# CFSAN-Biostatistics/snp-pipeline

Hardware: AMD Instinct MI355X
Metric: consensus_bases_called_per_sec (higher is better)
Workload: dtype u8; 1 GPU; BASELINE configs[3] shard (125 samples/GPU x 5000000 bp x 30x synthetic pileups, 49878 SNP sites, 1500 SNP records per sample; the reference bundles no pileups); step = site-record gather + site union, one batched scan launch + one call launch, 4-bit pack, row all-gather, all-pairs distance tiles, row-band exchange; samples_total=125, samples_this_rank=125, genome_bp=5000000, snp_sites=49878, pileup_bytes_this_rank=54061520755, parallelism=samples sharded over 1 rank(s)

## Files before the change

### include/snpgpu.h

```cpp
#ifndef SNPGPU_H
#define SNPGPU_H

#include <stddef.h>
#include <stdint.h>

#ifdef __cplusplus
extern "C" {
#endif

#define SNPGPU_ABI_VERSION 7

#define SNPGPU_OK            0
#define SNPGPU_E_HIP        -1
#define SNPGPU_E_ARG        -2
#define SNPGPU_E_NOMEM      -3
#define SNPGPU_E_PILEUP     -4
#define SNPGPU_E_UNSUPPORTED -5
#define SNPGPU_E_IO         -6
#define SNPGPU_E_TIMEOUT    -7

#define SNPGPU_F_RAWDPTH  0x01
#define SNPGPU_F_VARFREQ  0x02
#define SNPGPU_F_DEPTH    0x04
#define SNPGPU_F_STRDPTH  0x08
// ... 474 lines not shown
int  snpgpu_tiles_gather_dev(snpgpu_ctx *ctx, const int32_t *d_matrix, uint32_t n_padded, const uint32_t *d_tile_rows,
                             const uint32_t *d_tile_cols, uint32_t n_tiles, int32_t *d_out);
int  snpgpu_tiles_scatter_dev(snpgpu_ctx *ctx, const int32_t *d_tiles, const uint32_t *d_tile_rows, const uint32_t *d_tile_cols,
                              uint32_t n_tiles, int32_t *d_matrix, uint32_t n_padded);
int  snpgpu_group_check_dev(snpgpu_ctx *ctx, const uint8_t *d_filters, const snpgpu_site_counts *d_counts, const uint64_t *d_line_off,
                            const uint8_t *d_wanted, const uint32_t *d_excl_off, const uint32_t *d_excl_slots,
                            uint32_t n_samples, uint32_t n_sites, int64_t *d_out);

int  snpgpu_dense_windows(snpgpu_ctx *ctx, const int64_t *positions, const uint32_t *seg_off, uint32_t n_segs,
                          const int32_t *max_snps, const int32_t *window, uint32_t n_rules,
                          int64_t *out_start, int64_t *out_end, uint32_t *out_seg, uint32_t *out_n);
int  snpgpu_dense_windows_dev(snpgpu_ctx *ctx, const int64_t *d_positions, const uint32_t *d_seg_off, uint32_t n_segs,
                              uint32_t n_pos, const int32_t *max_snps , const int32_t *window ,
                              uint32_t n_rules, int64_t *d_out_start, int64_t *d_out_end, uint32_t *d_out_seg,
                              uint32_t *d_out_n );
int  snpgpu_merge_regions(snpgpu_ctx *ctx, const uint32_t *group, const int64_t *start, const int64_t *end,
                          uint32_t n, uint32_t *out_group, int64_t *out_start, int64_t *out_end, uint32_t *out_n);
int  snpgpu_merge_regions_dev(snpgpu_ctx *ctx, const uint32_t *d_group, const int64_t *d_start, const int64_t *d_end,
                              uint32_t n, uint32_t *d_out_group, int64_t *d_out_start, int64_t *d_out_end,
                              uint32_t *d_out_n );
int  snpgpu_in_regions(snpgpu_ctx *ctx, const uint32_t *pos_group, const int64_t *positions, uint32_t n_pos,
                       const uint32_t *reg_off, const int64_t *reg_start, const int64_t *reg_end,
                       uint32_t n_groups, uint8_t *out_flag);
int  snpgpu_in_regions_dev(snpgpu_ctx *ctx, const uint32_t *d_pos_group, const int64_t *d_positions, uint32_t n_pos,
                           const uint32_t *d_reg_off, const int64_t *d_reg_start, const int64_t *d_reg_end,
                           uint32_t n_groups, uint8_t *d_out_flag);

int  snpgpu_merge_sites(snpgpu_ctx *ctx, const uint64_t *keys, const uint32_t *sample_of_key, size_t n,
                        uint64_t *out_unique, uint32_t *out_off, uint32_t *out_carrier,
                        uint32_t *out_n_unique, uint32_t *out_n_carrier);
int  snpgpu_merge_sites_dev(snpgpu_ctx *ctx, const uint64_t *d_keys, const uint32_t *d_sample_of_key, uint32_t n,
                            uint64_t *d_out_unique, uint32_t *d_out_off, uint32_t *d_out_carrier,
                            uint32_t *d_out_n );

typedef struct snpgpu_synth_params {
    uint64_t seed;
    uint32_t sample;
    uint32_t genome_len;
    float    mean_depth;
    float    carrier_p_same_clade;
    float    carrier_p_other_clade;
    uint32_t n_clades;
    char     contig[32];
} snpgpu_synth_params;
int  snpgpu_synth_reference_dev(snpgpu_ctx *ctx, uint64_t seed, uint32_t genome_len, uint8_t *d_ref );
int  snpgpu_synth_pileup_dev(snpgpu_ctx *ctx, const snpgpu_synth_params *p, const uint8_t *d_ref,
                             const uint8_t *d_site_alt, uint8_t *d_out, size_t capacity, size_t *out_nbytes);

#define SNPGPU_BGZF_E_NOT_GZIP   -101
#define SNPGPU_BGZF_E_NOT_BGZF   -102
#define SNPGPU_BGZF_E_TRUNCATED  -103
#define SNPGPU_BGZF_E_ISIZE      -104
#define SNPGPU_BGZF_E_MAGIC      -105
#define SNPGPU_BGZF_ST_OK           0
#define SNPGPU_BGZF_ST_BTYPE        1
#define SNPGPU_BGZF_ST_STORED_LEN   2
#define SNPGPU_BGZF_ST_CODE_SET     3
#define SNPGPU_BGZF_ST_SYMBOL       4
#define SNPGPU_BGZF_ST_DISTANCE     5
#define SNPGPU_BGZF_ST_INPUT_END    6
#define SNPGPU_BGZF_ST_OUTPUT_OVER  7
#define SNPGPU_BGZF_ST_OUTPUT_SHORT 8
#define SNPGPU_BGZF_ST_CRC          9
typedef struct snpgpu_bgzf_block {
    uint64_t coff;
    uint64_t poff;
// ... 36 lines not shown
```

### snp_pipeline_amd/_lib.py

```python
import ctypes as C
import os

_HERE = os.path.dirname(os.path.abspath(__file__))
LIB_PATH = os.path.join(_HERE, "lib", "libsnpgpu.so")

MAX_SYMS = 8
SCAN_STATUS_WORDS = 4
CALL_PASSES = 4

F_RAWDPTH, F_VARFREQ, F_DEPTH, F_STRDPTH, F_STRBIAS, F_REGION = 1, 2, 4, 8, 16, 32
SITE_IN_SNPLIST, SITE_EXCLUDED = 1, 2
ST_NO_LINE, ST_OK, ST_SHORT_LINE, ST_BAD_DEPTH, ST_NO_QUALS, ST_MULTI_REF = 0, 1, 2, 3, 4, 5
VCF_LINE_WINDOW, VCF_MORE_UNUSUAL, VCF_LONG_LINE = 4096, 1, 2
E_HIP, E_ARG, E_NOMEM, E_PILEUP, E_UNSUPPORTED, E_IO, E_TIMEOUT = -1, -2, -3, -4, -5, -6, -7


class CallerParams(C.Structure):
    _fields_ = [("min_base_quality", C.c_int32), ("min_cons_depth", C.c_int32),
                ("min_cons_strand_depth", C.c_int32), ("reserved", C.c_int32),
                ("min_cons_freq", C.c_double), ("min_cons_strand_bias", C.c_double)]


class SiteCounts(C.Structure):
    _fields_ = [("raw_depth", C.c_uint32), ("good_depth", C.c_uint32), ("fwd_good_depth", C.c_uint32),
# ... 194 lines not shown
                                          C.c_int]),
    "snpgpu_pair_sites_kept": (C.c_int, [_P, _P, _P, C.c_uint64, C.c_uint64, _P, _P, _P, C.POINTER(C.c_uint64)]),
    "snpgpu_packed_drop": (C.c_int, [_P]),
    "snpgpu_write_pair_sites_tsv": (C.c_int, [C.c_char_p, _P, _P, C.c_uint32, _P, _P, C.c_uint64, _P, _P, _P, _P, _P, _P, _P]),
    "snpgpu_distance_rect_packed_dev": (C.c_int, [_P, _P, C.c_uint32, _P, C.c_uint32, C.c_uint32, C.c_int, _P, C.c_uint64]),
    "snpgpu_nearest_dev": (C.c_int, [_P, _P, C.c_uint32, C.c_uint32, C.c_uint64, C.c_uint32, C.c_int32, C.c_uint64, _P, _P, _P, C.POINTER(C.c_uint64)]),
    "snpgpu_nearest": (C.c_int, [_P, _P, C.c_uint32, _P, C.c_uint32, C.c_uint32, C.c_uint32, C.c_int32, C.c_uint32, C.c_int, C.c_uint64, _P, _P, _P,
                                 C.POINTER(C.c_uint64), _P]),
    "snpgpu_write_nearest_tsv": (C.c_int, [C.c_char_p, _P, _P, C.c_uint32, _P, _P, C.c_uint32, _P, _P, _P]),
    "snpgpu_valid_plane_row_bytes": (C.c_size_t, [C.c_uint32]),
    "snpgpu_valid_plane_dev": (C.c_int, [_P, _P, C.c_uint32, C.c_uint32, _P]),
    "snpgpu_compared_rect_dev": (C.c_int, [_P, _P, C.c_uint32, _P, C.c_uint32, C.c_uint32, _P, C.c_uint64]),
    "snpgpu_compared_pairs_dev": (C.c_int, [_P, _P, C.c_uint32, _P, C.c_uint32, C.c_uint32, _P, _P, C.c_uint64, _P]),
    "snpgpu_compared": (C.c_int, [_P, _P, C.c_uint32, C.c_uint32, _P]),
    "snpgpu_compared_pairs": (C.c_int, [_P, _P, C.c_uint32, _P, C.c_uint32, C.c_uint32, _P, _P, C.c_uint64, _P]),
    "snpgpu_write_pair_rows_tsv": (C.c_int, [C.c_char_p, _P, _P, C.c_uint32, _P, _P, C.c_uint32, _P, _P, _P, _P, C.c_uint64]),
    "snpgpu_site_counts_dev": (C.c_int, [_P, _P, C.c_uint32, C.c_uint32, _P]),
    "snpgpu_site_counts_host": (C.c_int, [_P, _P, C.c_uint32, C.c_uint32, _P]),
    "snpgpu_cluster_snps_dev": (C.c_int, [_P, _P, C.c_uint32, C.c_uint32, _P, C.c_uint32, C.c_uint64, _P, _P, _P, _P, C.POINTER(C.c_uint64)]),
    "snpgpu_cluster_snps": (C.c_int, [_P, _P, C.c_uint32, C.c_uint32, _P, _P, C.c_uint32, C.c_uint64, _P, _P, _P, _P, C.POINTER(C.c_uint64)]),
    "snpgpu_write_site_counts_tsv": (C.c_int, [C.c_char_p, _P, C.c_uint32, C.c_uint32, _P, _P, _P, _P]),
    "snpgpu_write_cluster_snps_tsv": (C.c_int, [C.c_char_p, _P, _P, C.c_uint32, _P, _P, _P, _P, _P, C.c_uint32, _P, _P, _P, _P]),
    "snpgpu_dense_windows": (C.c_int, [_P, _P, _P, C.c_uint32, _P, _P, C.c_uint32, _P, _P, _P, C.POINTER(C.c_uint32)]),
    "snpgpu_merge_regions": (C.c_int, [_P, _P, _P, _P, C.c_uint32, _P, _P, _P, C.POINTER(C.c_uint32)]),
    "snpgpu_in_regions": (C.c_int, [_P, _P, _P, C.c_uint32, _P, _P, _P, C.c_uint32, _P]),
    "snpgpu_merge_sites": (C.c_int, [_P, _P, _P, C.c_size_t, _P, _P, _P, C.POINTER(C.c_uint32), C.POINTER(C.c_uint32)]),
    "snpgpu_dense_windows_dev": (C.c_int, [_P, _P, _P, C.c_uint32, C.c_uint32, _P, _P, C.c_uint32, _P, _P, _P, _P]),
    "snpgpu_merge_regions_dev": (C.c_int, [_P, _P, _P, _P, C.c_uint32, _P, _P, _P, _P]),
    "snpgpu_in_regions_dev": (C.c_int, [_P, _P, _P, C.c_uint32, _P, _P, _P, C.c_uint32, _P]),
    "snpgpu_merge_vcf_files": (C.c_int, [_P, C.POINTER(C.c_char_p), C.c_uint32, C.c_char_p, C.c_char_p, C.c_uint32, C.c_uint32, _P]),
    "snpgpu_merge_vcf_files_opts": (C.c_int, [_P, C.POINTER(C.c_char_p), C.c_uint32, C.c_char_p, C.c_char_p, C.c_uint32, _P, _P, _P]),
    "snpgpu_merge_plan": (C.c_int, [C.c_uint32, C.c_uint64, C.c_uint64, _P, _P]),
    "snpgpu_merge_sites_dev": (C.c_int, [_P, _P, _P, C.c_uint32, _P, _P, _P, _P]),
    "snpgpu_comm_available": (C.c_int, []),
    "snpgpu_comm_version": (C.c_int, [C.POINTER(C.c_int)]),
    "snpgpu_comm_unique_id": (C.c_int, [_P]),
    "snpgpu_comm_init": (C.c_int, [_P, C.c_int, C.c_int, _P]),
    "snpgpu_comm_destroy": (None, [_P]),
    "snpgpu_comm_abort": (None, [_P]),
    "snpgpu_comm_info": (C.c_int, [_P, C.POINTER(C.c_int), C.POINTER(C.c_int), C.POINTER(C.c_int)]),
    "snpgpu_allgather": (C.c_int, [_P, _P, _P, C.c_size_t]),
    "snpgpu_allgatherv": (C.c_int, [_P, _P, _P, _P, _P]),
    "snpgpu_alltoallv": (C.c_int, [_P, _P, _P, _P, _P]),
    "snpgpu_stream_wait": (C.c_int, [_P, C.c_uint32]),
    "snpgpu_tiles_gather_dev": (C.c_int, [_P, _P, C.c_uint32, _P, _P, C.c_uint32, _P]),
    "snpgpu_tiles_scatter_dev": (C.c_int, [_P, _P, _P, _P, C.c_uint32, _P, C.c_uint32]),
    "snpgpu_group_check_dev": (C.c_int, [_P, _P, _P, _P, _P, _P, _P, C.c_uint32, C.c_uint32, _P]),
    "snpgpu_synth_reference_dev": (C.c_int, [_P, C.c_uint64, C.c_uint32, _P]),
    "snpgpu_synth_pileup_dev": (C.c_int, [_P, C.POINTER(SynthParams), _P, _P, _P, C.c_size_t, C.POINTER(C.c_size_t)]),
    "snpgpu_bgzf_probe": (C.c_int, [C.c_char_p]),
    "snpgpu_bgzf_strerror": (C.c_char_p, [C.c_int]),
    "snpgpu_bgzf_status_name": (C.c_char_p, [C.c_uint32]),
    "snpgpu_bgzf_index": (C.c_int, [_P, C.c_uint64, _P, C.c_uint64, C.POINTER(C.c_uint64), C.POINTER(BgzfInfo)]),
    "snpgpu_bgzf_inflate_dev": (C.c_int, [_P, _P, C.c_uint64, _P, C.c_uint64, _P, C.c_uint64, _P, C.POINTER(BgzfInfo)]),
    "snpgpu_bgzf_inflate_block_host": (C.c_uint32, [_P, C.POINTER(BgzfBlock), _P]),
    "snpgpu_bgzf_read_range": (C.c_int, [C.c_char_p, C.c_uint64, C.c_uint64, _P, C.POINTER(C.c_uint64)]),
    "snpgpu_call_consensus_bgzf_files": (C.c_int, [_P, _P, C.POINTER(C.c_char_p), C.c_uint32, C.POINTER(CallerParams), _P, _P, _P, _P,
                                                   _P, _P, _P, _P, C.POINTER(StreamOpts), C.POINTER(StreamStats), _P]),
}

_lib = None


class SnpGpuError(RuntimeError):
    def __init__(self, code, message):
        RuntimeError.__init__(self, "snpgpu error %d: %s" % (code, message))
# ... 27 lines not shown
```

### snp_pipeline_amd/csrc/regions.hip

```cpp
#include <string.h>

#include <vector>

#include "internal.h"
#include "prims.h"

namespace {

inline size_t up256(size_t x) { return (x + 255) / 256 * 256; }
inline unsigned nblk(uint64_t n) { return (unsigned)((n + 255) / 256); }

#define R_TRY(ctx, expr)                                                                                \
    do {                                                                                                \
        hipError_t e_ = (expr);                                                                         \
        if (e_ != hipSuccess)                                                                           \
            return snpgpu_set_error((ctx), SNPGPU_E_HIP, "%s failed: %s", #expr, hipGetErrorString(e_)); \
    } while (0)

#define REG_ERR_POSITION 1u
#define REG_ERR_INTERVAL 2u

struct U64Less { __device__ bool operator()(const uint64_t &a, const uint64_t &b) const { return a < b; } };

#define MAX_RULES 64
struct Rules { int32_t max_snps[MAX_RULES], window[MAX_RULES]; uint32_t n; };

__device__ __forceinline__ uint32_t seg_of(const uint32_t *seg_off, uint32_t n_segs, uint32_t i) {
    uint32_t lo = 0, hi = n_segs;
    while (hi - lo > 1) { uint32_t mid = (lo + hi) >> 1; if (seg_off[mid] <= i) lo = mid; else hi = mid; }
    return lo;
}

// ... 146 lines not shown
        k_ival_pack<<<nblk(n), 256, 0, st>>>(d_group, d_start, d_end, n, iv, d_out_n);
        const Ival *sorted = prim_sort<Ival, IvalLess>(st, iv, ia, ib, n, sflag, IvalLess());
        k_ival_ends<<<nblk(n), 256, 0, st>>>(sorted, n, gm);
        prim_inclusive_scan<GroupMax, GroupMaxOp>(st, gm, run, n, aggr, GroupMaxOp());
        k_ival_heads<<<nblk(n), 256, 0, st>>>(sorted, run, n, head);
        uint32_t *d_total = nullptr;
        prim_exclusive_scan_u32(st, head, slot, n, scan_ws, &d_total);
        k_ival_emit<<<nblk(n), 256, 0, st>>>(sorted, run, head, slot, n, d_out_group, d_out_start, d_out_end);
        k_copy_word<<<1, 1, 0, st>>>(d_total, d_out_n);
    }
    R_TRY(ctx, hipGetLastError());
    return SNPGPU_OK;
}

__global__ void k_in_regions(const uint32_t *pos_group, const int64_t *pos, uint32_t n, const uint32_t *reg_off,
                             const int64_t *rs, const int64_t *re, uint32_t n_groups, uint8_t *out) {
    uint32_t i = blockIdx.x * blockDim.x + threadIdx.x;
    if (i >= n) return;
    uint32_t g = pos_group[i];
    uint8_t f = 0;
    if (g < n_groups) {
        int64_t p = pos[i];
        uint32_t lo = reg_off[g], hi = reg_off[g + 1];
        while (lo < hi) {
            uint32_t mid = (lo + hi) >> 1;
            if (rs[mid] <= p) lo = mid + 1; else hi = mid;
        }
        if (lo > reg_off[g]) f = re[lo - 1] >= p;
    }
    out[i] = f;
}

struct Pair { uint64_t key; uint32_t samp, pad; };
struct PairLess {
    __device__ bool operator()(const Pair &a, const Pair &b) const { return a.key != b.key ? a.key < b.key : a.samp < b.samp; }
};

__global__ void k_pair_pack(const uint64_t *keys, const uint32_t *samp, uint32_t n, Pair *out) {
    uint32_t i = blockIdx.x * blockDim.x + threadIdx.x;
    if (i < n) { Pair p; p.key = keys[i]; p.samp = samp[i]; p.pad = 0; out[i] = p; }
}

__global__ void k_sites_flags(const Pair *sorted, uint32_t n, uint32_t *new_key, uint32_t *new_pair) {
    uint32_t i = blockIdx.x * blockDim.x + threadIdx.x;
    if (i >= n) return;
    const bool nk = i == 0 || sorted[i].key != sorted[i - 1].key;
    new_key[i] = nk;
    new_pair[i] = nk || sorted[i].samp != sorted[i - 1].samp;
}

__global__ void k_sites_emit(const Pair *sorted, uint32_t n, const uint32_t *new_key, const uint32_t *new_pair, const uint32_t *key_slot,
                             const uint32_t *pair_slot, const uint32_t *n_keys, const uint32_t *n_pairs, uint64_t *out_unique,
                             uint32_t *out_off, uint32_t *out_carrier, uint32_t *out_n) {
    uint32_t i = blockIdx.x * blockDim.x + threadIdx.x;
    if (i == 0) { out_n[0] = *n_keys; out_n[1] = *n_pairs; out_off[*n_keys] = *n_pairs; }
    if (i >= n) return;
    if (new_pair[i]) out_carrier[pair_slot[i]] = sorted[i].samp;
    if (new_key[i]) { out_unique[key_slot[i]] = sorted[i].key; out_off[key_slot[i]] = pair_slot[i]; }
}

size_t merge_sites_ws_bytes(uint64_t n) {
    return 3 * up256(sizeof(Pair) * (size_t)n) + 256 + 4 * up256(4ull * n) + 2 * up256(4 * prim_scan_workspace_words(n)) + 256;
}

int merge_sites_enqueue(snpgpu_ctx *ctx, const uint64_t *d_keys, const uint32_t *d_samp, uint32_t n, uint64_t *d_out_unique,
                        uint32_t *d_out_off, uint32_t *d_out_carrier, uint32_t *d_out_n, char *ws) {
    hipStream_t st = ctx->stream;
    size_t o = 0;
    Pair *pr = (Pair *)(ws + o); o += up256(sizeof(Pair) * (size_t)n);
    Pair *pa = (Pair *)(ws + o); o += up256(sizeof(Pair) * (size_t)n);
    Pair *pb = (Pair *)(ws + o); o += up256(sizeof(Pair) * (size_t)n);
    uint32_t *sflag = (uint32_t *)(ws + o); o += 256;
    uint32_t *nk = (uint32_t *)(ws + o); o += up256(4ull * n);
    uint32_t *np = (uint32_t *)(ws + o); o += up256(4ull * n);
    uint32_t *ks = (uint32_t *)(ws + o); o += up256(4ull * n);
    uint32_t *ps = (uint32_t *)(ws + o); o += up256(4ull * n);
    uint32_t *scan1 = (uint32_t *)(ws + o); o += up256(4 * prim_scan_workspace_words(n));
    uint32_t *scan2 = (uint32_t *)(ws + o);
    R_TRY(ctx, hipMemsetAsync(d_out_n, 0, 8, st));
    R_TRY(ctx, hipMemsetAsync(d_out_off, 0, 4, st));
    if (n) {
        k_pair_pack<<<nblk(n), 256, 0, st>>>(d_keys, d_samp, n, pr);
        const Pair *sorted = prim_sort<Pair, PairLess>(st, pr, pa, pb, n, sflag, PairLess());
        k_sites_flags<<<nblk(n), 256, 0, st>>>(sorted, n, nk, np);
        uint32_t *t_keys = nullptr, *t_pairs = nullptr;
        prim_exclusive_scan_u32(st, nk, ks, n, scan1, &t_keys);
        prim_exclusive_scan_u32(st, np, ps, n, scan2, &t_pairs);
        k_sites_emit<<<nblk(n), 256, 0, st>>>(sorted, n, nk, np, ks, ps, t_keys, t_pairs, d_out_unique, d_out_off, d_out_carrier, d_out_n);
    }
    R_TRY(ctx, hipGetLastError());
    return SNPGPU_OK;
}

int region_error(snpgpu_ctx *ctx, uint32_t bits) {
    if (bits & REG_ERR_POSITION) return snpgpu_set_error(ctx, SNPGPU_E_UNSUPPORTED, "SNP position outside [0, 2^40)");
    if (bits & REG_ERR_INTERVAL) return snpgpu_set_error(ctx, SNPGPU_E_UNSUPPORTED, "interval with start > end");
    return SNPGPU_OK;
}

}

extern "C" {

int snpgpu_dense_windows_dev(snpgpu_ctx *ctx, const int64_t *d_positions, const uint32_t *d_seg_off, uint32_t n_segs, uint32_t n_pos,
                             const int32_t *max_snps, const int32_t *window, uint32_t n_rules, int64_t *d_out_start,
                             int64_t *d_out_end, uint32_t *d_out_seg, uint32_t *d_out_n) {
    if (!ctx || !d_out_n) return SNPGPU_E_ARG;
    Rules rules;
    int rc = make_rules(ctx, max_snps, window, n_rules, rules);
    if (rc) return rc;
    if ((uint64_t)n_pos * n_rules > 0x7FFFFFFFull) return snpgpu_set_error(ctx, SNPGPU_E_UNSUPPORTED, "too many (position, rule) pairs");
    if (n_segs >= (1u << 24)) return snpgpu_set_error(ctx, SNPGPU_E_UNSUPPORTED, "too many segments");
    if (n_pos && (!d_positions || !d_seg_off || !d_out_start || !d_out_end || !d_out_seg)) return snpgpu_set_error(ctx, SNPGPU_E_ARG, "null dense-window argument");
    R_TRY(ctx, snpgpu_enter(ctx));
    void *ws = nullptr;
    rc = snpgpu_scratch(ctx, dense_ws_bytes(n_pos, n_rules), &ws);
    if (rc) return rc;
    return dense_enqueue(ctx, d_positions, d_seg_off, n_segs, n_pos, rules, d_out_start, d_out_end, d_out_seg, d_out_n, (char *)ws);
}

int snpgpu_merge_regions_dev(snpgpu_ctx *ctx, const uint32_t *d_group, const int64_t *d_start, const int64_t *d_end, uint32_t n,
                             uint32_t *d_out_group, int64_t *d_out_start, int64_t *d_out_end, uint32_t *d_out_n) {
    if (!ctx || !d_out_n) return SNPGPU_E_ARG;
    if (n && (!d_group || !d_start || !d_end || !d_out_group || !d_out_start || !d_out_end)) return snpgpu_set_error(ctx, SNPGPU_E_ARG, "null merge argument");
    R_TRY(ctx, snpgpu_enter(ctx));
    void *ws = nullptr;
    int rc = snpgpu_scratch(ctx, merge_regions_ws_bytes(n), &ws);
    if (rc) return rc;
    return merge_regions_enqueue(ctx, d_group, d_start, d_end, n, d_out_group, d_out_start, d_out_end, d_out_n, (char *)ws);
}

int snpgpu_in_regions_dev(snpgpu_ctx *ctx, const uint32_t *d_pos_group, const int64_t *d_positions, uint32_t n_pos,
                          const uint32_t *d_reg_off, const int64_t *d_reg_start, const int64_t *d_reg_end, uint32_t n_groups,
                          uint8_t *d_out_flag) {
    if (!ctx) return SNPGPU_E_ARG;
    if (n_pos == 0) return SNPGPU_OK;
    if (!d_pos_group || !d_positions || !d_out_flag || (n_groups && !d_reg_off)) return snpgpu_set_error(ctx, SNPGPU_E_ARG, "null in_regions argument");
    R_TRY(ctx, snpgpu_enter(ctx));
    k_in_regions<<<nblk(n_pos), 256, 0, ctx->stream>>>(d_pos_group, d_positions, n_pos, d_reg_off, d_reg_start, d_reg_end, n_groups, d_out_flag);
    R_TRY(ctx, hipGetLastError());
    return SNPGPU_OK;
}

int snpgpu_merge_sites_dev(snpgpu_ctx *ctx, const uint64_t *d_keys, const uint32_t *d_sample_of_key, uint32_t n,
                           uint64_t *d_out_unique, uint32_t *d_out_off, uint32_t *d_out_carrier, uint32_t *d_out_n) {
    if (!ctx || !d_out_n || !d_out_off) return SNPGPU_E_ARG;
    if (n > 0x7FFFFFFFu) return snpgpu_set_error(ctx, SNPGPU_E_UNSUPPORTED, "too many site records");
    if (n && (!d_keys || !d_sample_of_key || !d_out_unique || !d_out_carrier)) return snpgpu_set_error(ctx, SNPGPU_E_ARG, "null merge_sites argument");
    R_TRY(ctx, snpgpu_enter(ctx));
    void *ws = nullptr;
    int rc = snpgpu_scratch(ctx, merge_sites_ws_bytes(n), &ws);
    if (rc) return rc;
    return merge_sites_enqueue(ctx, d_keys, d_sample_of_key, n, d_out_unique, d_out_off, d_out_carrier, d_out_n, (char *)ws);
}

int snpgpu_dense_windows(snpgpu_ctx *ctx, const int64_t *positions, const uint32_t *seg_off, uint32_t n_segs,
                         const int32_t *max_snps, const int32_t *window, uint32_t n_rules,
                         int64_t *out_start, int64_t *out_end, uint32_t *out_seg, uint32_t *out_n) {
    if (!ctx || !out_n) return SNPGPU_E_ARG;
    *out_n = 0;
    if (n_segs == 0 || n_rules == 0) return SNPGPU_OK;
    if (!seg_off) return snpgpu_set_error(ctx, SNPGPU_E_ARG, "null dense-window argument");
    const uint32_t n_pos = seg_off[n_segs];
    if (n_pos == 0) return SNPGPU_OK;
    if (!positions || !out_start || !out_end || !out_seg) return snpgpu_set_error(ctx, SNPGPU_E_ARG, "null dense-window argument");
    Rules rules;
    int rc = make_rules(ctx, max_snps, window, n_rules, rules);
    if (rc) return rc;
    const uint64_t total = (uint64_t)n_pos * n_rules;
    if (total > 0x7FFFFFFFull) return snpgpu_set_error(ctx, SNPGPU_E_UNSUPPORTED, "too many (position, rule) pairs");
    if (n_segs >= (1u << 24)) return snpgpu_set_error(ctx, SNPGPU_E_UNSUPPORTED, "too many segments");
    R_TRY(ctx, snpgpu_enter(ctx));
    hipStream_t st = ctx->stream;
    size_t o = 0;
    const size_t o_pos = o; o += up256(8ull * n_pos);
    const size_t o_seg = o; o += up256(4ull * (n_segs + 1));
    const size_t o_os = o; o += up256(8 * total);
    const size_t o_oe = o; o += up256(8 * total);
    const size_t o_og = o; o += up256(4 * total);
    const size_t o_n = o; o += 256;
    const size_t o_ws = o; o += dense_ws_bytes(n_pos, n_rules);
    void *scr = nullptr;
    rc = snpgpu_scratch(ctx, o, &scr);
    if (rc) return rc;
    char *b = (char *)scr;
    R_TRY(ctx, hipMemcpyAsync(b + o_pos, positions, 8ull * n_pos, hipMemcpyHostToDevice, st));
// ... 142 lines not shown
```

Measured before the change: 713.0 million bases/s.

## Add sample-sort fast path for site union on small record counts

Adds a four-kernel sample sort for merge_sites when the record count fits a fixed cap. Each tile is sorted and deduplicated in LDS, samples pick 256 bucket splitters, each bucket is merged and run-length flagged in LDS, and a final kernel scatters unique keys, offsets and carriers. This replaces the generic multi-pass radix/pair sort and scan sequence with fewer launches and on-chip work. The cost is a complex new code path with capacity caps that must hold; it can be turned off through an environment variable.

Result: no change. 718.2 million bases/s (median of 6 runs) (+0.7%).

```diff
diff --git a/include/snpgpu.h b/include/snpgpu.h
--- a/include/snpgpu.h
+++ b/include/snpgpu.h
@@ -530,6 +530,7 @@
 int  snpgpu_merge_sites_dev(snpgpu_ctx *ctx, const uint64_t *d_keys, const uint32_t *d_sample_of_key, uint32_t n,
                             uint64_t *d_out_unique, uint32_t *d_out_off, uint32_t *d_out_carrier,
                             uint32_t *d_out_n );
+void snpgpu_site_union_params(uint32_t out[5]);
 
 typedef struct snpgpu_synth_params {
     uint64_t seed;
diff --git a/snp_pipeline_amd/_lib.py b/snp_pipeline_amd/_lib.py
--- a/snp_pipeline_amd/_lib.py
+++ b/snp_pipeline_amd/_lib.py
@@ -250,6 +250,7 @@
     "snpgpu_merge_vcf_files_opts": (C.c_int, [_P, C.POINTER(C.c_char_p), C.c_uint32, C.c_char_p, C.c_char_p, C.c_uint32, _P, _P, _P]),
     "snpgpu_merge_plan": (C.c_int, [C.c_uint32, C.c_uint64, C.c_uint64, _P, _P]),
     "snpgpu_merge_sites_dev": (C.c_int, [_P, _P, _P, C.c_uint32, _P, _P, _P, _P]),
+    "snpgpu_site_union_params": (None, [C.POINTER(C.c_uint32)]),
     "snpgpu_comm_available": (C.c_int, []),
     "snpgpu_comm_version": (C.c_int, [C.POINTER(C.c_int)]),
     "snpgpu_comm_unique_id": (C.c_int, [_P]),
diff --git a/snp_pipeline_amd/csrc/regions.hip b/snp_pipeline_amd/csrc/regions.hip
--- a/snp_pipeline_amd/csrc/regions.hip
+++ b/snp_pipeline_amd/csrc/regions.hip
@@ -1,3 +1,4 @@
+#include <stdlib.h>
 #include <string.h>
 
 #include <vector>
@@ -237,13 +238,321 @@
     if (new_key[i]) { out_unique[key_slot[i]] = sorted[i].key; out_off[key_slot[i]] = pair_slot[i]; }
 }
 
+#define SU_TILE 4096u
+#define SU_STRIDE 64u
+#define SU_BUCKETS 256u
+#define SU_FAST_MAX 262144u
+#define SU_THREADS 1024u
+#define SU_WAVES (SU_THREADS / 64)
+#define SU_TILE_SAMPLES (SU_TILE / SU_STRIDE)
+#define SU_TILES_MAX (SU_FAST_MAX / SU_TILE)
+#define SU_SAMPLES_MAX (SU_TILES_MAX * SU_TILE_SAMPLES)
+#define SU_Q_MAX ((SU_SAMPLES_MAX + SU_BUCKETS - 1) / SU_BUCKETS)
+#define SU_BUCKET_CAP ((SU_Q_MAX + SU_TILES_MAX) * SU_STRIDE)
+static_assert(SU_FAST_MAX % SU_TILE == 0 && SU_TILE % SU_STRIDE == 0, "whole tiles, whole sample strides");
+static_assert(SU_TILES_MAX <= 64, "k_su_splitters and k_su_buckets give every tile a lane of one wave");
+static_assert(SU_TILE_SAMPLES == 64, "k_su_splitters gives every sample of a tile a lane");
+static_assert(SU_BUCKETS == 256, "k_su_emit sums the buckets' counts with a thread per bucket");
+static_assert(SU_BUCKET_CAP * 12 + 2048 <= 65536 && SU_TILE * 12 + 256 <= 65536 && SU_SAMPLES_MAX * 12 + 8192 <= 65536, "static LDS");
+
+template <int R>
+__device__ __forceinline__ void su_merge_sort(uint64_t *key, uint32_t *samp, uint32_t cnt) {
+    for (uint32_t L = 1; L < cnt; L <<= 1) {
+        uint64_t K[R];
+        uint32_t S[R], to[R];
+#pragma unroll
+        for (int r = 0; r < R; ++r) {
+            const uint32_t i = threadIdx.x + r * SU_THREADS;
+            to[r] = i; K[r] = 0; S[r] = 0;
+            if (i < cnt) {
+                const uint32_t base = i & ~(2 * L - 1), mid = base + L, end = base + 2 * L < cnt ? base + 2 * L : cnt;
+                const uint64_t k = key[i];
+                const uint32_t s = samp[i];
+                K[r] = k; S[r] = s;
+                if (mid < end) {
+                    const uint64_t lk = key[mid - 1], rk = key[mid];
+                    if (rk < lk || (rk == lk && samp[mid] < samp[mid - 1])) {
+                        uint32_t lo = i < mid ? mid : base, hi = i < mid ? end : mid;
+                        const uint32_t eq = i < mid ? 0u : 1u;
+                        while (lo < hi) {
+                            const uint32_t m = (lo + hi) >> 1;
+                            const uint64_t mk = key[m];
+                            if (mk < k || (mk == k && (eq ? samp[m] <= s : samp[m] < s))) lo = m + 1; else hi = m;
+                        }
+                        to[r] = i < mid ? i + (lo - mid) : i - L + (lo - base);
+                    }
+                }
+            }
+        }
+        __syncthreads();
+#pragma unroll
+        for (int r = 0; r < R; ++r) {
+            const uint32_t i = threadIdx.x + r * SU_THREADS;
+            if (i < cnt && to[r] != i) { key[to[r]] = K[r]; samp[to[r]] = S[r]; }
+        }
+        __syncthreads();
+    }
+}
+
+__global__ __launch_bounds__(SU_THREADS) void k_su_tiles(const uint64_t *keys, const uint32_t *samp, uint32_t n, uint64_t *tile_key, uint32_t *tile_samp,
+                                                         uint32_t *tile_len, uint64_t *smp_key, uint32_t *smp_samp) {
+    __shared__ uint64_t lk[SU_TILE];
+    __shared__ uint32_t ls[SU_TILE];
+    __shared__ uint32_t sums[17];
+    const uint32_t base = blockIdx.x * SU_TILE;
+    const uint32_t cnt = n - base < SU_TILE ? n - base : SU_TILE;
+    for (uint32_t i = threadIdx.x; i < cnt; i += SU_THREADS) { lk[i] = keys[base + i]; ls[i] = samp[base + i]; }
+    __syncthreads();
+    su_merge_sort<SU_TILE / SU_THREADS>(lk, ls, cnt);
+    uint32_t kept = 0;
+    for (uint32_t r0 = 0; r0 < cnt; r0 += SU_THREADS) {
+        const uint32_t i = r0 + threadIdx.x;
+        uint64_t k = 0;
+        uint32_t s = 0, f = 0;
+        if (i < cnt) { k = lk[i]; s = ls[i]; f = i == 0 || k != lk[i - 1] || s != ls[i - 1]; }
+        uint32_t total;
+        const uint32_t pos = kept + block_exclusive_sum(f, sums, total);
+        if (f) {
+            tile_key[base + pos] = k; tile_samp[base + pos] = s;
+            if (pos % SU_STRIDE == 0) { smp_key[blockIdx.x * SU_TILE_SAMPLES + pos / SU_STRIDE] = k; smp_samp[blockIdx.x * SU_TILE_SAMPLES + pos / SU_STRIDE] = s; }
+        }
+        kept += total;
+        __syncthreads();
+    }
+    if (threadIdx.x == 0) tile_len[blockIdx.x] = kept;
+}
+
+__global__ __launch_bounds__(SU_THREADS) void k_su_splitters(const uint32_t *tile_len, uint32_t n_tiles, const uint64_t *smp_key, const uint32_t *smp_samp,
+                                                             uint64_t *spl_key, uint32_t *spl_samp, uint32_t *spl_tile) {
+    __shared__ uint64_t lk[SU_SAMPLES_MAX];
+    __shared__ uint32_t ls[SU_SAMPLES_MAX];
+    __shared__ uint32_t run_len[64], part[SU_WAVES][64], n_samples;
+    const uint32_t tile = blockIdx.x, wave = threadIdx.x >> 6, lane = threadIdx.x & 63;
+    if (threadIdx.x < 64) {
+        const uint32_t c = threadIdx.x < n_tiles ? (tile_len[threadIdx.x] + SU_STRIDE - 1) / SU_STRIDE : 0u;
+        const uint32_t incl = wave_inclusive_sum(c);
+        run_len[threadIdx.x] = c;
+        if (threadIdx.x == 63) n_samples = incl;
+    }
+    for (uint32_t i = threadIdx.x; i < n_tiles * SU_TILE_SAMPLES; i += SU_THREADS)
+        if ((i % SU_TILE_SAMPLES) * SU_STRIDE < tile_len[i / SU_TILE_SAMPLES]) { lk[i] = smp_key[i]; ls[i] = smp_samp[i]; }
+    __syncthreads();
+    const bool mine = lane < run_len[tile];
+    const uint64_t k = mine ? lk[tile * SU_TILE_SAMPLES + lane] : 0;
+    const uint32_t s = mine ? ls[tile * SU_TILE_SAMPLES + lane] : 0;
+    uint32_t before = 0;
+    if (mine)
+        for (uint32_t other = wave; other < n_tiles; other += SU_WAVES) {
+            uint32_t lo = 0, hi = run_len[other];
+            if (other == tile) { lo = hi = lane; }
+            const uint64_t *ok = lk + other * SU_TILE_SAMPLES;
+            const uint32_t *os = ls + other * SU_TILE_SAMPLES;
+            while (lo < hi) {
+                const uint32_t m = (lo + hi) >> 1;
+                if (ok[m] < k || (ok[m] == k && (other < tile ? os[m] <= s : os[m] < s))) lo = m + 1; else hi = m;
+            }
+            before += lo;
+        }
+    part[wave][lane] = before;
+    __syncthreads();
+    const uint32_t m = n_samples, q = (m + SU_BUCKETS - 1) / SU_BUCKETS;
+    if (threadIdx.x < 64 && mine) {
+        uint32_t rank = 0;
+        for (uint32_t w = 0; w < SU_WAVES; ++w) rank += part[w][lane];
+        if (rank && rank % q == 0 && rank / q < SU_BUCKETS) { spl_key[rank / q] = k; spl_samp[rank / q] = s; spl_tile[rank / q] = tile; }
+    }
+    if (tile == 0)
+        for (uint32_t b = threadIdx.x + 1; b < SU_BUCKETS; b += SU_THREADS)
+            if (b * q >= m) { spl_key[b] = ~0ull; spl_samp[b] = ~0u; spl_tile[b] = ~0u; }
+}
+
+
+
+__device__ __forceinline__ bool su_is_before(uint64_t k, uint32_t s, uint32_t tile, uint64_t sk, uint32_t ss, uint32_t st) {
+    return k < sk || (k == sk && (s < ss || (s == ss && tile < st)));
+}
+
+#define SU_TILES_PER_WAVE ((SU_TILES_MAX + SU_WAVES - 1) / SU_WAVES)
+static_assert(SU_TILE_SAMPLES <= 64 && SU_STRIDE <= 64, "a wave looks at a tile's samples, then at the elements between two, at once");
+
+__global__ __launch_bounds__(SU_THREADS) void k_su_buckets(const uint64_t *tile_key, const uint32_t *tile_samp, const uint32_t *tile_len, uint32_t n_tiles,
+                                                           const uint64_t *smp_key, const uint32_t *smp_samp, const uint64_t *spl_key, const uint32_t *spl_samp, const uint32_t *spl_tile,
+                                                           uint64_t *bkt_key, uint32_t *bkt_samp, uint32_t *bkt_slot, uint32_t *bkt_start, uint32_t *bkt_pairs, uint32_t *bkt_keys, uint32_t n) {
+    __shared__ uint64_t lk[SU_BUCKET_CAP];
+    __shared__ uint32_t ls[SU_BUCKET_CAP];
+    __shared__ uint32_t p_lo[64], p_hi[64], p_off[65], sums[17];
+    __shared__ uint64_t pred_key;
+    __shared__ uint32_t pred_samp, pred_any, start_all;
+    const uint32_t b = blockIdx.x, wave = threadIdx.x >> 6, lane = threadIdx.x & 63;
+    uint64_t sk[2];
+    uint32_t ss[2], st[2];
+#pragma unroll
+    for (int e = 0; e < 2; ++e) {
+        const bool real = b + e >= 1 && b + e < SU_BUCKETS;
+        sk[e] = real ? spl_key[b + e] : 0; ss[e] = real ? spl_samp[b + e] : 0; st[e] = real ? spl_tile[b + e] : 0;
+    }
+    uint32_t lo[SU_TILES_PER_WAVE][2], hi[SU_TILES_PER_WAVE][2];
+#pragma unroll
+    for (int x = 0; x < SU_TILES_PER_WAVE; ++x) {
+        const uint32_t tile = wave + SU_WAVES * x, len = tile < n_tiles ? tile_len[tile] : 0u;
+#pragma unroll
+        for (int e = 0; e < 2; ++e) {
+            const bool search = e == 0 ? b != 0 : b != SU_BUCKETS - 1;
+            bool before = false;
+            if (search && lane * SU_STRIDE < len)
+                before = su_is_before(smp_key[tile * SU_TILE_SAMPLES + lane], smp_samp[tile * SU_TILE_SAMPLES + lane], tile, sk[e], ss[e], st[e]);
+            const uint32_t c = (uint32_t)__popcll(__ballot(before));
+            lo[x][e] = c ? (c - 1) * SU_STRIDE + 1 : 0u;
+            hi[x][e] = c ? (c * SU_STRIDE < len ? c * SU_STRIDE : len) : 0u;
+            if (!search) lo[x][e] = hi[x][e] = e == 0 ? 0u : len;
+        }
+    }
+#pragma unroll
+    for (int x = 0; x < SU_TILES_PER_WAVE; ++x)
+#pragma unroll
+        for (int e = 0; e < 2; ++e) {
+            const uint32_t tile = wave + SU_WAVES * x, at = lo[x][e] + lane;
+            bool before = false;
+            if (at < hi[x][e]) before = su_is_before(tile_key[(size_t)tile * SU_TILE + at], tile_samp[(size_t)tile * SU_TILE + at], tile, sk[e], ss[e], st[e]);
+            lo[x][e] += (uint32_t)__popcll(__ballot(before));
+        }
+    if (lane == 0) {
+#pragma unroll
+        for (int x = 0; x < SU_TILES_PER_WAVE; ++x) {
+            const uint32_t tile = wave + SU_WAVES * x;
+            if (tile < 64) { p_lo[tile] = lo[x][0]; p_hi[tile] = lo[x][1] > lo[x][0] ? lo[x][1] : lo[x][0]; }
+        }
+    }
+    __syncthreads();
+    if (threadIdx.x < 64) {
+        const uint32_t i = threadIdx.x, l = p_lo[i], c = p_hi[i] - l;
+        const uint32_t incl = wave_inclusive_sum(c), before = wave_inclusive_sum(l);
+        p_off[i] = incl - c;
+        unsigned long long pk = 0;
+        uint32_t ps = 0, any = l > 0;
+        if (any) { pk = tile_key[(size_t)i * SU_TILE + l - 1]; ps = tile_samp[(size_t)i * SU_TILE + l - 1]; }
+        for (int dd = 32; dd > 0; dd >>= 1) {
+            const unsigned long long ok = __shfl_xor(pk, dd);
+            const uint32_t os = __shfl_xor(ps, dd), oa = __shfl_xor(any, dd);
+            if (oa && (!any || ok > pk || (ok == pk && os > ps))) { pk = ok; ps = os; any = 1; }
+        }
+        if (i == 63) { p_off[64] = incl; start_all = before; pred_key = pk; pred_samp = ps; pred_any = any; }
+    }
+    __syncthreads();
+    const uint32_t cnt = p_off[64] < SU_BUCKET_CAP ? p_off[64] : SU_BUCKET_CAP;
+    for (uint32_t tile = wave; tile < n_tiles; tile += SU_WAVES) {
+        const uint32_t l = p_lo[tile], off = p_off[tile], c = p_off[tile + 1] - off;
+        for (uint32_t e = lane; e < c; e += 64)
+            if (off + e < SU_BUCKET_CAP) { lk[off + e] = tile_key[(size_t)tile * SU_TILE + l + e]; ls[off + e] = tile_samp[(size_t)tile * SU_TILE + l + e]; }
+    }
+    __syncthreads();
+    su_merge_sort<SU_BUCKET_CAP / SU_THREADS>(lk, ls, cnt);
+    const uint32_t start = start_all;
+    uint32_t n_pairs = 0, n_keys = 0;
+    for (uint32_t r0 = 0; r0 < cnt; r0 += SU_THREADS) {
+        const uint32_t e = r0 + threadIdx.x;
+        uint32_t new_pair = 0, new_key = 0, s = 0;
+        uint64_t k = 0;
+        if (e < cnt) {
+            k = lk[e]; s = ls[e];
+            const bool has = e > 0 || pred_any;
+            const uint64_t pk = e > 0 ? lk[e - 1] : pred_key;
+            const uint32_t ps = e > 0 ? ls[e - 1] : pred_samp;
+            new_key = !has || k != pk;
+            new_pair = new_key || s != ps;
+        }
+        uint32_t total;
+        const uint32_t pos = block_exclusive_sum(new_pair | (new_key << 16), sums, total);
+        if (new_pair) {
+            const uint32_t j = start + n_pairs + (pos & 0xFFFFu);
+            if (j < n) { bkt_key[j] = k; bkt_samp[j] = s; bkt_slot[j] = (n_keys + (pos >> 16)) | (new_key << 31); }
+        }
+        n_pairs += total & 0xFFFFu; n_keys += total >> 16;
+        __syncthreads();
+    }
+    if (threadIdx.x == 0) { bkt_start[b] = start; bkt_pairs[b] = n_pairs; bkt_keys[b] = n_keys; }
+}
+
+__global__ __launch_bounds__(SU_BUCKETS) void k_su_emit(const uint64_t *bkt_key, const uint32_t *bkt_samp, const uint32_t *bkt_slot, const uint32_t *bkt_start,
+                                                        const uint32_t *bkt_pairs, const uint32_t *bkt_keys, uint64_t *out_unique, uint32_t *out_off,
+                                                        uint32_t *out_carrier, uint32_t *out_n, uint32_t n) {
+    __shared__ uint32_t sums[17];
+    const uint32_t b = blockIdx.x, upto = b == 0 ? SU_BUCKETS : b;
+    uint32_t pairs_before, keys_before;
+    block_exclusive_sum(threadIdx.x < upto ? bkt_pairs[threadIdx.x] : 0u, sums, pairs_before);
+    __syncthreads();
+    block_exclusive_sum(threadIdx.x < upto ? bkt_keys[threadIdx.x] : 0u, sums, keys_before);
+    if (b == 0) {
+        if (threadIdx.x == 0) { out_n[0] = keys_before; out_n[1] = pairs_before; if (keys_before <= n) out_off[keys_before] = pairs_before; }
+        pairs_before = keys_before = 0;
+    }
+    const uint32_t start = bkt_start[b], n_pairs = bkt_pairs[b];
+    for (uint32_t j = threadIdx.x; j < n_pairs; j += SU_BUCKETS) {
+        if (start + j >= n || pairs_before + j >= n) continue;
+        const uint32_t slot = bkt_slot[start + j];
+        out_carrier[pairs_before + j] = bkt_samp[start + j];
+        const uint32_t u = keys_before + (slot & 0x7FFFFFFFu);
+        if ((slot >> 31) && u < n) { out_unique[u] = bkt_key[start + j]; out_off[u] = pairs_before + j; }
+    }
+}
+
+__global__ void k_su_empty(uint32_t *out_off, uint32_t *out_n) { out_n[0] = 0; out_n[1] = 0; out_off[0] = 0; }
+
+struct SuWs { size_t tile_key, tile_samp, tile_len, smp_key, smp_samp, spl_key, spl_samp, spl_tile, bkt_key, bkt_samp, bkt_slot, bkt_start, bkt_pairs, bkt_keys, bytes; };
+SuWs su_ws(uint64_t n) {
+    const size_t tiles = (size_t)((n + SU_TILE - 1) / SU_TILE);
+    SuWs w;
+    size_t o = 0;
+    w.tile_key = o; o += up256(8ull * n);
+    w.bkt_key = o; o += up256(8ull * n);
+    w.smp_key = o; o += up256(8 * tiles * SU_TILE_SAMPLES);
+    w.spl_key = o; o += up256(8 * SU_BUCKETS);
+    w.tile_samp = o; o += up256(4ull * n);
+    w.bkt_samp = o; o += up256(4ull * n);
+    w.bkt_slot = o; o += up256(4ull * n);
+    w.smp_samp = o; o += up256(4 * tiles * SU_TILE_SAMPLES);
+    w.tile_len = o; o += up256(4 * SU_TILES_MAX);
+    w.spl_samp = o; o += up256(4 * SU_BUCKETS);
+    w.spl_tile = o; o += up256(4 * SU_BUCKETS);
+    w.bkt_start = o; o += up256(4 * SU_BUCKETS);
+    w.bkt_pairs = o; o += up256(4 * SU_BUCKETS);
+    w.bkt_keys = o; o += up256(4 * SU_BUCKETS);
+    w.bytes = o;
+    return w;
+}
+
+bool su_forced_general() {
+    const char *e = getenv("SNPGPU_SITE_UNION");
+    return e && strcmp(e, "general") == 0;
+}
+
 size_t merge_sites_ws_bytes(uint64_t n) {
-    return 3 * up256(sizeof(Pair) * (size_t)n) + 256 + 4 * up256(4ull * n) + 2 * up256(4 * prim_scan_workspace_words(n)) + 256;
+    const size_t general = 3 * up256(sizeof(Pair) * (size_t)n) + 256 + 4 * up256(4ull * n) + 2 * up256(4 * prim_scan_workspace_words(n)) + 256;
+    const size_t fast = n <= SU_FAST_MAX ? su_ws(n).bytes : 0;
+    return general > fast ? general : fast;
 }
 
 int merge_sites_enqueue(snpgpu_ctx *ctx, const uint64_t *d_keys, const uint32_t *d_samp, uint32_t n, uint64_t *d_out_unique,
                         uint32_t *d_out_off, uint32_t *d_out_carrier, uint32_t *d_out_n, char *ws) {
     hipStream_t st = ctx->stream;
+    if (n <= SU_FAST_MAX && !su_forced_general()) {
+        if (n == 0) {
+            k_su_empty<<<1, 1, 0, st>>>(d_out_off, d_out_n);
+        } else {
+            const SuWs w = su_ws(n);
+            const uint32_t tiles = (n + SU_TILE - 1) / SU_TILE;
+            uint64_t *tile_key = (uint64_t *)(ws + w.tile_key), *smp_key = (uint64_t *)(ws + w.smp_key), *spl_key = (uint64_t *)(ws + w.spl_key), *bkt_key = (uint64_t *)(ws + w.bkt_key);
+            uint32_t *tile_samp = (uint32_t *)(ws + w.tile_samp), *tile_len = (uint32_t *)(ws + w.tile_len), *smp_samp = (uint32_t *)(ws + w.smp_samp);
+            uint32_t *spl_samp = (uint32_t *)(ws + w.spl_samp), *spl_tile = (uint32_t *)(ws + w.spl_tile), *bkt_samp = (uint32_t *)(ws + w.bkt_samp), *bkt_slot = (uint32_t *)(ws + w.bkt_slot);
+            uint32_t *bkt_start = (uint32_t *)(ws + w.bkt_start), *bkt_pairs = (uint32_t *)(ws + w.bkt_pairs), *bkt_keys = (uint32_t *)(ws + w.bkt_keys);
+            k_su_tiles<<<tiles, SU_THREADS, 0, st>>>(d_keys, d_samp, n, tile_key, tile_samp, tile_len, smp_key, smp_samp);
+            k_su_splitters<<<tiles, SU_THREADS, 0, st>>>(tile_len, tiles, smp_key, smp_samp, spl_key, spl_samp, spl_tile);
+            k_su_buckets<<<SU_BUCKETS, SU_THREADS, 0, st>>>(tile_key, tile_samp, tile_len, tiles, smp_key, smp_samp, spl_key, spl_samp, spl_tile, bkt_key, bkt_samp, bkt_slot, bkt_start, bkt_pairs, bkt_keys, n);
+            k_su_emit<<<SU_BUCKETS, SU_BUCKETS, 0, st>>>(bkt_key, bkt_samp, bkt_slot, bkt_start, bkt_pairs, bkt_keys, d_out_unique, d_out_off, d_out_carrier, d_out_n, n);
+        }
+        R_TRY(ctx, hipGetLastError());
+        return SNPGPU_OK;
+    }
     size_t o = 0;
     Pair *pr = (Pair *)(ws + o); o += up256(sizeof(Pair) * (size_t)n);
     Pair *pa = (Pair *)(ws + o); o += up256(sizeof(Pair) * (size_t)n);
@@ -330,6 +639,10 @@
     int rc = snpgpu_scratch(ctx, merge_sites_ws_bytes(n), &ws);
     if (rc) return rc;
     return merge_sites_enqueue(ctx, d_keys, d_sample_of_key, n, d_out_unique, d_out_off, d_out_carrier, d_out_n, (char *)ws);
+}
+
+void snpgpu_site_union_params(uint32_t out[5]) {
+    out[0] = SU_TILE; out[1] = SU_STRIDE; out[2] = SU_BUCKETS; out[3] = SU_FAST_MAX; out[4] = SU_BUCKET_CAP;
 }
 
 int snpgpu_dense_windows(snpgpu_ctx *ctx, const int64_t *positions, const uint32_t *seg_off, uint32_t n_segs,
```

## Replace generic sort and full-length scans in site union with tiled bitonic merge pipeline

Applied to the files above, without the earlier changes.

Site-union merging now uses its own sort. A shared-memory bitonic sort runs per 4096-element tile, then merge-path passes with wave-ballot split search, replacing the generic prim_sort and the pair-pack kernel. Flag computation and the two full-length exclusive scans become per-block packed counts with a small block-level scan, and emit then writes outputs directly. This cuts kernel launches, global passes and workspace, but the 16-bit packed counters assume at most 2048 items per block, and the new code is custom and harder to verify.

Result: no change. 704.2 million bases/s before, 709.0 million bases/s after (median of 6 runs) (+0.7%).

```diff
diff --git a/snp_pipeline_amd/csrc/regions.hip b/snp_pipeline_amd/csrc/regions.hip
--- a/snp_pipeline_amd/csrc/regions.hip
+++ b/snp_pipeline_amd/csrc/regions.hip
@@ -210,62 +210,215 @@
 }
 
 struct Pair { uint64_t key; uint32_t samp, pad; };
-struct PairLess {
-    __device__ bool operator()(const Pair &a, const Pair &b) const { return a.key != b.key ? a.key < b.key : a.samp < b.samp; }
-};
-
-__global__ void k_pair_pack(const uint64_t *keys, const uint32_t *samp, uint32_t n, Pair *out) {
-    uint32_t i = blockIdx.x * blockDim.x + threadIdx.x;
-    if (i < n) { Pair p; p.key = keys[i]; p.samp = samp[i]; p.pad = 0; out[i] = p; }
-}
-
-__global__ void k_sites_flags(const Pair *sorted, uint32_t n, uint32_t *new_key, uint32_t *new_pair) {
-    uint32_t i = blockIdx.x * blockDim.x + threadIdx.x;
+__device__ __forceinline__ bool pair_less(const Pair &a, const Pair &b) { return a.key != b.key ? a.key < b.key : a.samp < b.samp; }
+
+#define SITES_THREADS 1024
+#define SITES_TILE 4096
+#define SITES_BLOCK 2048
+
+struct SiteRec { uint32_t lo, hi, samp; };
+__device__ __forceinline__ bool site_less(const SiteRec &a, const SiteRec &b) {
+    const uint64_t ka = (uint64_t)a.hi << 32 | a.lo, kb = (uint64_t)b.hi << 32 | b.lo;
+    return (ka < kb) | ((ka == kb) & (a.samp < b.samp));
+}
+__device__ __forceinline__ void site_cmpx(SiteRec &a, SiteRec &b, bool on) {
+    const bool sw = on & site_less(b, a);
+    const SiteRec x = a, y = b;
+    a.lo = sw ? y.lo : x.lo; a.hi = sw ? y.hi : x.hi; a.samp = sw ? y.samp : x.samp;
+    b.lo = sw ? x.lo : y.lo; b.hi = sw ? x.hi : y.hi; b.samp = sw ? x.samp : y.samp;
+}
+__device__ __forceinline__ uint32_t site_slot(uint32_t i) { return i ^ ((i >> 5 & 1u) * 21u) ^ ((i >> 6 & 1u) * 26u); }
+
+__global__ __launch_bounds__(SITES_THREADS) void k_sites_tile_sort(const uint64_t *keys, const uint32_t *samp, uint32_t n, Pair *out,
+                                                                  uint32_t *out_n, uint32_t *out_off) {
+    __shared__ uint32_t key_lo[SITES_TILE], key_hi[SITES_TILE], smp[SITES_TILE];
+    const uint32_t t = threadIdx.x;
+    const uint32_t base = blockIdx.x * SITES_TILE;
+    const uint32_t cnt = n - base < SITES_TILE ? n - base : SITES_TILE;
+    if (blockIdx.x == 0 && t == 0) { out_n[0] = 0; out_n[1] = 0; out_off[0] = 0; }
+    for (uint32_t i = t; i < SITES_TILE; i += SITES_THREADS) {
+        const bool in = i < cnt;
+        const uint64_t k = in ? keys[base + i] : 0ull;
+        const uint32_t p = site_slot(i);
+        key_lo[p] = (uint32_t)k; key_hi[p] = (uint32_t)(k >> 32); smp[p] = in ? samp[base + i] : 0u;
+    }
+    __syncthreads();
+    auto load = [&](uint32_t p) -> SiteRec { SiteRec r; r.lo = key_lo[p]; r.hi = key_hi[p]; r.samp = smp[p]; return r; };
+    auto store = [&](uint32_t p, const SiteRec &r) { key_lo[p] = r.lo; key_hi[p] = r.hi; smp[p] = r.samp; };
+    auto two_stages = [&](uint32_t a0, uint32_t a1, uint32_t a2, uint32_t a3, bool mirror) {
+        const uint32_t p0 = site_slot(a0), p1 = site_slot(a1), p2 = site_slot(a2), p3 = site_slot(a3);
+        const bool on1 = a1 < cnt, on2 = a2 < cnt, on3 = a3 < cnt;
+        SiteRec e0 = load(p0), e1 = load(p1), e2 = load(p2), e3 = load(p3);
+        if (mirror) { site_cmpx(e0, e3, on3); site_cmpx(e1, e2, on2); }
+        else { site_cmpx(e0, e2, on2); site_cmpx(e1, e3, on3); }
+        site_cmpx(e0, e1, on1); site_cmpx(e2, e3, on3);
+        store(p0, e0); store(p1, e1); store(p2, e2); store(p3, e3);
+        __syncthreads();
+    };
+    auto stride_one = [&]() {
+        const uint32_t a0 = t << 2;
+        const uint32_t p0 = site_slot(a0), p1 = site_slot(a0 | 1), p2 = site_slot(a0 | 2), p3 = site_slot(a0 | 3);
+        SiteRec e0 = load(p0), e1 = load(p1), e2 = load(p2), e3 = load(p3);
+        site_cmpx(e0, e1, (a0 | 1) < cnt); site_cmpx(e2, e3, (a0 | 3) < cnt);
+        store(p0, e0); store(p1, e1); store(p2, e2); store(p3, e3);
+        __syncthreads();
+    };
+    stride_one();
+    for (uint32_t k = 4; k <= SITES_TILE; k <<= 1) {
+        uint32_t jl = k >> 2;
+        uint32_t a0 = ((t & ~(jl - 1)) << 2) | (t & (jl - 1));
+        two_stages(a0, a0 | jl, a0 ^ (k - 1) ^ jl, a0 ^ (k - 1), true);
+        uint32_t j = k >> 3;
+        for (; j >= 2; j >>= 2) {
+            jl = j >> 1;
+            a0 = ((t & ~(jl - 1)) << 2) | (t & (jl - 1));
+            two_stages(a0, a0 | jl, a0 | j, a0 | j | jl, false);
+        }
+        if (j == 1) stride_one();
+    }
+    for (uint32_t i = t; i < cnt; i += SITES_THREADS) {
+        const uint32_t p = site_slot(i);
+        Pair r; r.key = ((uint64_t)key_hi[p] << 32) | key_lo[p]; r.samp = smp[p]; r.pad = 0;
+        out[base + i] = r;
+    }
+}
+
+__device__ __forceinline__ uint32_t sites_split(const Pair *A, uint32_t a_len, const Pair *B, uint32_t b_len, uint32_t d) {
+    const uint32_t lane = threadIdx.x & 63;
+    uint32_t lo = d > b_len ? d - b_len : 0, hi = d < a_len ? d : a_len;
+    while (lo < hi) {
+        const uint32_t step = (hi - lo + 63) >> 6;
+        const uint32_t mid = lo + (lane + 1) * step - 1;
+        const bool first = mid < hi && !pair_less(B[d - 1 - mid], A[mid]);
+        const uint32_t c = (uint32_t)__popcll(__ballot(first));
+        const uint32_t end = lo + (c + 1) * step - 1;
+        lo += c * step;
+        hi = end < hi ? end : hi;
+    }
+    return lo;
+}
+
+__global__ __launch_bounds__(SITES_THREADS) void k_sites_merge(const Pair *in, Pair *out, uint32_t n, uint32_t run) {
+    __shared__ Pair stage[SITES_BLOCK];
+    __shared__ uint32_t split[2];
+    const uint32_t o0 = blockIdx.x * SITES_BLOCK;
+    const uint32_t pair0 = o0 / (2 * run) * (2 * run);
+    const uint32_t a_len = n - pair0 < run ? n - pair0 : run;
+    const uint32_t b_begin = pair0 + a_len, b_len = n - b_begin < run ? n - b_begin : run;
+    const uint32_t d0 = o0 - pair0, total = a_len + b_len;
+    const uint32_t d1 = d0 + SITES_BLOCK < total ? d0 + SITES_BLOCK : total;
+    const Pair *A = in + pair0, *B = in + b_begin;
+    const uint32_t wave = threadIdx.x >> 6;
+    if (wave < 2) {
+        const uint32_t s = sites_split(A, a_len, B, b_len, wave ? d1 : d0);
+        if ((threadIdx.x & 63) == 0) split[wave] = s;
+    }
+    __syncthreads();
+    const uint32_t a0 = split[0], a1 = split[1], b0 = d0 - a0, b1 = d1 - a1;
+    const uint32_t na = a1 - a0, nb = b1 - b0;
+    for (uint32_t i = threadIdx.x; i < na + nb; i += SITES_THREADS) stage[i] = i < na ? A[a0 + i] : B[b0 + (i - na)];
+    __syncthreads();
+    for (uint32_t i = threadIdx.x; i < na + nb; i += SITES_THREADS) {
+        const Pair v = stage[i];
+        uint32_t lo = 0, hi;
+        if (i < na) {
+            hi = nb;
+            while (lo < hi) { const uint32_t mid = (lo + hi) >> 1; if (pair_less(stage[na + mid], v)) lo = mid + 1; else hi = mid; }
+            out[o0 + i + lo] = v;
+        } else {
+            hi = na;
+            while (lo < hi) { const uint32_t mid = (lo + hi) >> 1; if (!pair_less(v, stage[mid])) lo = mid + 1; else hi = mid; }
+            out[o0 + (i - na) + lo] = v;
+        }
+    }
+}
+
+__device__ __forceinline__ void sites_flags(const Pair *sorted, uint32_t n, uint32_t i, Pair &r0, Pair &r1, uint32_t &f0, uint32_t &f1) {
+    f0 = f1 = 0;
     if (i >= n) return;
-    const bool nk = i == 0 || sorted[i].key != sorted[i - 1].key;
-    new_key[i] = nk;
-    new_pair[i] = nk || sorted[i].samp != sorted[i - 1].samp;
-}
-
-__global__ void k_sites_emit(const Pair *sorted, uint32_t n, const uint32_t *new_key, const uint32_t *new_pair, const uint32_t *key_slot,
-                             const uint32_t *pair_slot, const uint32_t *n_keys, const uint32_t *n_pairs, uint64_t *out_unique,
-                             uint32_t *out_off, uint32_t *out_carrier, uint32_t *out_n) {
-    uint32_t i = blockIdx.x * blockDim.x + threadIdx.x;
-    if (i == 0) { out_n[0] = *n_keys; out_n[1] = *n_pairs; out_off[*n_keys] = *n_pairs; }
-    if (i >= n) return;
-    if (new_pair[i]) out_carrier[pair_slot[i]] = sorted[i].samp;
-    if (new_key[i]) { out_unique[key_slot[i]] = sorted[i].key; out_off[key_slot[i]] = pair_slot[i]; }
-}
+    r0 = sorted[i];
+    Pair prev = r0;
+    if (i > 0) prev = sorted[i - 1];
+    const bool k0 = i == 0 || prev.key != r0.key;
+    f0 = (uint32_t)k0 | (uint32_t)(k0 || prev.samp != r0.samp) << 16;
+    if (i + 1 >= n) return;
+    r1 = sorted[i + 1];
+    const bool k1 = r1.key != r0.key;
+    f1 = (uint32_t)k1 | (uint32_t)(k1 || r1.samp != r0.samp) << 16;
+}
+
+__global__ __launch_bounds__(SITES_THREADS) void k_sites_count(const Pair *sorted, uint32_t n, uint32_t *blk_keys, uint32_t *blk_pairs) {
+    __shared__ uint32_t lds[17];
+    Pair r0, r1;
+    uint32_t f0, f1, total;
+    sites_flags(sorted, n, blockIdx.x * SITES_BLOCK + 2 * threadIdx.x, r0, r1, f0, f1);
+    (void)block_exclusive_sum(f0 + f1, lds, total);
+    if (threadIdx.x == 0) { blk_keys[blockIdx.x] = total & 0xFFFFu; blk_pairs[blockIdx.x] = total >> 16; }
+}
+
+__global__ __launch_bounds__(SITES_THREADS) void k_sites_emit(const Pair *sorted, uint32_t n, const uint32_t *blk_keys, const uint32_t *blk_pairs,
+                                                             uint32_t scanned, uint64_t *out_unique, uint32_t *out_off,
+                                                             uint32_t *out_carrier, uint32_t *out_n) {
+    __shared__ uint32_t lds_k[17], lds_p[17], lds_f[17];
+    uint32_t key0, pair0;
+    if (scanned) {
+        key0 = blk_keys[blockIdx.x]; pair0 = blk_pairs[blockIdx.x];
+    } else {
+        const bool before = threadIdx.x < blockIdx.x;
+        (void)block_exclusive_sum(before ? blk_keys[threadIdx.x] : 0u, lds_k, key0);
+        (void)block_exclusive_sum(before ? blk_pairs[threadIdx.x] : 0u, lds_p, pair0);
+    }
+    Pair r0, r1;
+    uint32_t f0, f1, total;
+    sites_flags(sorted, n, blockIdx.x * SITES_BLOCK + 2 * threadIdx.x, r0, r1, f0, f1);
+    const uint32_t ex = block_exclusive_sum(f0 + f1, lds_f, total);
+    uint32_t ks = key0 + (ex & 0xFFFFu), ps = pair0 + (ex >> 16);
+    if (f0 >> 16) out_carrier[ps] = r0.samp;
+    if (f0 & 1u) { out_unique[ks] = r0.key; out_off[ks] = ps; }
+    ks += f0 & 1u; ps += f0 >> 16;
+    if (f1 >> 16) out_carrier[ps] = r1.samp;
+    if (f1 & 1u) { out_unique[ks] = r1.key; out_off[ks] = ps; }
+    if (blockIdx.x == gridDim.x - 1 && threadIdx.x == 0) {
+        const uint32_t n_keys = key0 + (total & 0xFFFFu), n_pairs = pair0 + (total >> 16);
+        out_n[0] = n_keys; out_n[1] = n_pairs; out_off[n_keys] = n_pairs;
+    }
+}
+
+inline uint32_t sites_blocks(uint64_t n) { return (uint32_t)((n + SITES_BLOCK - 1) / SITES_BLOCK); }
 
 size_t merge_sites_ws_bytes(uint64_t n) {
-    return 3 * up256(sizeof(Pair) * (size_t)n) + 256 + 4 * up256(4ull * n) + 2 * up256(4 * prim_scan_workspace_words(n)) + 256;
+    const uint32_t nb = sites_blocks(n);
+    return 2 * up256(sizeof(Pair) * (size_t)n) + 2 * up256(4ull * nb) + 2 * up256(4 * prim_scan_workspace_words(nb));
 }
 
 int merge_sites_enqueue(snpgpu_ctx *ctx, const uint64_t *d_keys, const uint32_t *d_samp, uint32_t n, uint64_t *d_out_unique,
                         uint32_t *d_out_off, uint32_t *d_out_carrier, uint32_t *d_out_n, char *ws) {
     hipStream_t st = ctx->stream;
     size_t o = 0;
-    Pair *pr = (Pair *)(ws + o); o += up256(sizeof(Pair) * (size_t)n);
-    Pair *pa = (Pair *)(ws + o); o += up256(sizeof(Pair) * (size_t)n);
-    Pair *pb = (Pair *)(ws + o); o += up256(sizeof(Pair) * (size_t)n);
-    uint32_t *sflag = (uint32_t *)(ws + o); o += 256;
-    uint32_t *nk = (uint32_t *)(ws + o); o += up256(4ull * n);
-    uint32_t *np = (uint32_t *)(ws + o); o += up256(4ull * n);
-    uint32_t *ks = (uint32_t *)(ws + o); o += up256(4ull * n);
-    uint32_t *ps = (uint32_t *)(ws + o); o += up256(4ull * n);
-    uint32_t *scan1 = (uint32_t *)(ws + o); o += up256(4 * prim_scan_workspace_words(n));
+    const uint32_t nb = sites_blocks(n);
+    Pair *src = (Pair *)(ws + o); o += up256(sizeof(Pair) * (size_t)n);
+    Pair *dst = (Pair *)(ws + o); o += up256(sizeof(Pair) * (size_t)n);
+    uint32_t *bk = (uint32_t *)(ws + o); o += up256(4ull * nb);
+    uint32_t *bp = (uint32_t *)(ws + o); o += up256(4ull * nb);
+    uint32_t *scan1 = (uint32_t *)(ws + o); o += up256(4 * prim_scan_workspace_words(nb));
     uint32_t *scan2 = (uint32_t *)(ws + o);
-    R_TRY(ctx, hipMemsetAsync(d_out_n, 0, 8, st));
-    R_TRY(ctx, hipMemsetAsync(d_out_off, 0, 4, st));
-    if (n) {
-        k_pair_pack<<<nblk(n), 256, 0, st>>>(d_keys, d_samp, n, pr);
-        const Pair *sorted = prim_sort<Pair, PairLess>(st, pr, pa, pb, n, sflag, PairLess());
-        k_sites_flags<<<nblk(n), 256, 0, st>>>(sorted, n, nk, np);
-        uint32_t *t_keys = nullptr, *t_pairs = nullptr;
-        prim_exclusive_scan_u32(st, nk, ks, n, scan1, &t_keys);
-        prim_exclusive_scan_u32(st, np, ps, n, scan2, &t_pairs);
-        k_sites_emit<<<nblk(n), 256, 0, st>>>(sorted, n, nk, np, ks, ps, t_keys, t_pairs, d_out_unique, d_out_off, d_out_carrier, d_out_n);
-    }
+    if (n == 0) {
+        R_TRY(ctx, hipMemsetAsync(d_out_n, 0, 8, st));
+        R_TRY(ctx, hipMemsetAsync(d_out_off, 0, 4, st));
+        return SNPGPU_OK;
+    }
+    k_sites_tile_sort<<<(n + SITES_TILE - 1) / SITES_TILE, SITES_THREADS, 0, st>>>(d_keys, d_samp, n, src, d_out_n, d_out_off);
+    for (uint64_t run = SITES_TILE; run < n; run <<= 1) {
+        k_sites_merge<<<nb, SITES_THREADS, 0, st>>>(src, dst, n, (uint32_t)run);
+        Pair *t = src; src = dst; dst = t;
+    }
+    k_sites_count<<<nb, SITES_THREADS, 0, st>>>(src, n, bk, bp);
+    const bool scanned = nb > SITES_THREADS;
+    if (scanned) {
+        prim_exclusive_scan_u32(st, bk, bk, nb, scan1, nullptr);
+        prim_exclusive_scan_u32(st, bp, bp, nb, scan2, nullptr);
+    }
+    k_sites_emit<<<nb, SITES_THREADS, 0, st>>>(src, n, bk, bp, scanned, d_out_unique, d_out_off, d_out_carrier, d_out_n);
     R_TRY(ctx, hipGetLastError());
     return SNPGPU_OK;
 }
```
